# RoyAPTX4869/RaLD

Hardware: AMD Instinct MI355X
Metric: denoising steps/sec (whole node) (higher is better)
Workload: dtype bf16

## Files before the change

### include/rald_hip.h

```cpp
#ifndef RALD_HIP_H
#define RALD_HIP_H
#include <stdint.h>
#ifdef __cplusplus
extern "C" {
#endif

const char* rald_last_error(void);
int rald_version(void);
int rald_build_flags(void);
int64_t rald_debug_f16_saturation_count(int32_t reset);
int rald_debug_poison_lds(void* stream);

typedef struct rald_dit rald_dit;

typedef struct rald_dit_config {
    int32_t n_latents;
    int32_t channels;
    int32_t depth;
    int32_t n_heads;
    int32_t d_head;
    int32_t t_channels;
    int32_t context_dim;
    int32_t n_cond_tokens;
    int32_t with_radar_enc;
    int32_t enc_hidden_ch;
    int32_t enc_radar_ch;
    int32_t radar_r, radar_a, radar_e;
    float sigma_data;
    int32_t qkv_dtype;
} rald_dit_config;

void rald_dit_default_config(rald_dit_config* cfg);
int rald_dit_create(const rald_dit_config* cfg, rald_dit** out);
void rald_dit_destroy(rald_dit* h);
int rald_dit_load_weight(rald_dit* h, const char* name, const float* data, int64_t nelem);
int rald_dit_finalize(rald_dit* h);
int rald_dit_reserve(rald_dit* h, int32_t max_batch);
int64_t rald_dit_workspace_generation(const rald_dit* h);
int rald_dit_set_two_stream_min_batch(rald_dit* h, int32_t min_batch);
int32_t rald_dit_two_stream_min_batch(const rald_dit* h);

int rald_dit_set_sigmas(rald_dit* h, const float* sigmas_host, int32_t n, void* stream);

int64_t rald_dit_cond_cache_bytes(const rald_dit* h, int32_t batch);
int rald_dit_encode_cond_tokens(rald_dit* h, const float* tokens, int32_t batch, void* cond_cache, void* stream);
int rald_dit_encode_cond(rald_dit* h, const float* cube, int32_t batch, float* out_tokens, void* cond_cache, void* stream);

int rald_dit_denoise(rald_dit* h, const float* x, int32_t batch, int32_t sigma_row, int32_t per_sample,
                     const void* cond_cache, float* out, int32_t raw_F, void* stream);

int rald_dit_sample(rald_dit* h, const float* latents, int32_t batch, const void* cond_cache, int32_t num_steps,
                    float sigma_min, float sigma_max, float rho, float* out, void* stream);

int rald_edm_schedule(int32_t num_steps, double sigma_min, double sigma_max, double rho, double S_churn, double S_min, double S_max, float* t,
                      float* t_hat);
int rald_dit_sample_stochastic(rald_dit* h, const float* latents, int32_t batch, const void* cond_cache, int32_t num_steps, double sigma_min,
                               double sigma_max, double rho, double S_churn, double S_min, double S_max, double S_noise, const float* noise,
                               const int64_t* seeds, float* out, void* stream);
int rald_op_philox_normal(const int64_t* seeds, int32_t B, int64_t n_per_sample, int32_t tag, int32_t step, float* out, void* stream);

int rald_dit_profile_begin(rald_dit* h);
int rald_dit_profile_end(rald_dit* h, double* total_ms, int32_t* launches);
int rald_dit_profile_end_kinds(rald_dit* h, double* total_ms4, int32_t* launches4);
int rald_dit_profile_set_kinds(rald_dit* h, uint32_t kind_mask);

typedef struct rald_ae rald_ae;
typedef struct rald_ae_config {
    int32_t dim;
    int32_t num_latents;
    int32_t latent_dim;
    int32_t depth;
    int32_t heads;
    int32_t dim_head;
// ... 187 lines not shown
int rald_op_conv_pack_weights(const float* W, void* out_bf16, int32_t Cout, int32_t Cin, int32_t pad_to, int32_t dgrad, void* stream);
int rald_op_groupnorm(const float* x, const float* gamma, const float* beta, void* y_bf16, double* stats, int32_t B, int32_t S, int32_t C,
                      int32_t swish, void* stream);
int64_t rald_op_groupnorm_bwd_scratch_bytes(int32_t B, int32_t S, int32_t C);
int rald_op_groupnorm_bwd(const float* x, const double* stats, const float* gamma, const float* beta, const void* da, int32_t da_is_bf16, float* dx,
                          void* dx_bf16, float* dgamma, float* dbeta, double* gsum_scratch, int32_t B, int32_t S, int32_t C, int32_t swish,
                          int32_t accumulate, void* stream);
int rald_op_groupnorm_apply(const float* x, const double* stats, const float* gamma, const float* beta, void* y_bf16, int32_t B, int32_t S, int32_t C,
                            int32_t swish, void* stream);
int rald_op_conv_in(const float* cube, int32_t cube_ch, int32_t Cin, const float* W, const float* bias, float* out, int32_t B, int32_t D, int32_t H,
                    int32_t Wd, int32_t Cout, void* stream);
int rald_op_pad_channels(const float* x, void* out_bf16, int64_t M, int32_t C, int32_t Cpad, void* stream);
int rald_op_zero_insert2(const float* dy, void* out_bf16, int32_t B, int32_t OD, int32_t OH, int32_t OW, int32_t C, void* stream);
int rald_op_rowdot(const void* a_bf16, const void* b_bf16, int64_t M, int32_t C, float* out, void* stream);
int rald_op_softmax_rows(const float* S, int64_t ld_s, void* P_bf16, int64_t ld_p, int32_t rows, int32_t n, void* stream);
int rald_op_attn_self_proj(const void* qkv_bf16, int64_t ld, const void* Wo_bf16, float* part, int32_t n_latents, int32_t heads, int32_t batch,
                           void* stream);
int rald_op_xattn_q2_proj(const void* h_bf16, const void* Wq_bf16, const void* Kc_bf16, int64_t ldk, int64_t strideK, const void* Vt_bf16,
                          int64_t ldvt, int64_t strideVt, const void* Wo_bf16, float* part, int32_t M, int32_t n_latents, int32_t heads,
                          int32_t n_keys, float qscale, void* stream);
int rald_op_attn_self_proj_slabs(const void* qkv_bf16, int64_t ld, const void* Wo_bf16, void* part, int32_t n_latents, int32_t heads, int32_t batch,
                                 int32_t part_f16, void* stream);
int rald_op_xattn_q2_proj_slabs(const void* h_bf16, const void* Wq_bf16, const void* Kc_bf16, int64_t ldk, int64_t strideK, const void* Vt_bf16,
                                int64_t ldvt, int64_t strideVt, const void* Wo_bf16, void* part, int32_t M, int32_t n_latents, int32_t heads,
                                int32_t n_keys, float qscale, int32_t part_f16, void* stream);
int rald_op_reduce_resid_ln_slabs(const void* part, int32_t slabs, int64_t slab_stride, const float* bias, float* x, void* h_bf16, int32_t M,
                                  const float* g, const float* b, int64_t gstride, int32_t rows_per_group, float add_one, float eps, int32_t part_f16,
                                  void* stream);
int64_t rald_debug_f16_saturation_attn(int32_t reset);
int rald_op_proj_in(const float* xin, const float* W, float* x, int32_t M, int32_t C, int32_t D, const float* coef, int32_t coef_stride,
                    int32_t rows_per_group, void* stream);
int rald_op_final_norm_proj(const float* x, const float* gamma, const float* beta, const float* Wout, const float* xin, float* out, int32_t M,
                            int32_t D, int32_t C, const float* coef, int32_t coef_stride, int32_t rows_per_group, void* stream);
int rald_op_reduce_resid_ln(const float* part, int32_t slabs, int64_t slab_stride, const float* bias, float* x, void* h_bf16, int32_t M,
                            const float* g, const float* b, int64_t gstride, int32_t rows_per_group, float add_one, float eps, void* stream);
int rald_op_ae_decode_tables(int32_t dim, const float* wq, const float* wk, const float* norm_w, const float* norm_b, const float* wpe,
                             const float* bpe, const float* wfold, float* t2aug_out, uint16_t* l_img_out);
int64_t rald_op_ae_decode_scratch_bytes(int32_t batch, int32_t num_latents);
int rald_op_ae_decode(const float* x, const float* gamma, const float* beta, const float* t2aug, const uint16_t* l_img, const float* basis,
                      float c0, const float* queries, float* out_logits, int32_t batch, int64_t n_queries, int32_t num_latents, int32_t dim,
                      void* scratch, int64_t scratch_bytes, void* stream);
int rald_op_ae_cast_rays(const float* x, const float* gamma, const float* beta, const float* t2aug, const uint16_t* l_img, const float* basis,
                         float c0, const float* origins, const float* dirs, int64_t ray_batch_stride, int32_t n_steps, int32_t n_refine,
                         float* out_t, float* out_logit, int32_t* out_step, float* out_points, int32_t batch, int64_t n_rays,
                         int32_t num_latents, int32_t dim, void* scratch, int64_t scratch_bytes, void* stream);
int rald_op_ae_decode_grad(const float* x, const float* gamma, const float* beta, const float* t2aug, const uint16_t* l_img, const float* basis,
                           float c0, const float* queries, const int64_t* offsets, float* out_logits, float* out_grad, float* out_projected,
                           float max_step, int32_t batch, int64_t n_queries, int32_t num_latents, int32_t dim, void* scratch,
                           int64_t scratch_bytes, void* stream);
int rald_op_ae_encode_tables(int32_t dim, int32_t num_latents, int32_t heads, int32_t mix, const float* const* in, float* const* out);
int rald_op_ae_enc_features(const float* pc, const float* basis, const float* var_factor, void* F_f16, void* G_f16, int32_t batch, int32_t n_points,
                            int32_t rows_per_sample, void* stream);
int rald_op_ae_enc_qproj(const float* xin, const float* X0, float* x, const float* gamma, const float* beta, const float* T1, float* Q,
                         int32_t rows, int32_t num_latents, int32_t dim, void* stream);
int rald_op_attention_f16kv(const float* Q, int64_t ldq, int64_t strideQ, const void* KV_f16, void* O_bf16, int64_t ldo, int64_t strideO, int32_t nq,
                            int32_t nk, int32_t k_rows, int32_t heads, int32_t batch, int32_t ksplit, void* scratch, void* stream);
int rald_op_gemm_mx8(const void* A8, const void* scaleA, int64_t lda, int64_t strideA, int64_t strideSA, const void* B8, const void* scaleB,
                     int64_t ldb, int64_t strideB, int64_t strideSB, void* C, int64_t ldc, int64_t strideC, const float* bias, int32_t M,
                     int32_t N, int32_t K, int32_t batch, float alpha, int32_t epilogue, void* stream);
int rald_op_quantize_mx8(const void* in, int32_t in_is_bf16, int64_t ld_in, void* out_e4m3, int64_t ld_out, void* out_scales_e8m0, int64_t rows,
                         int32_t K, void* stream);
int rald_op_layernorm_mx8(const float* x, void* out_e4m3, void* out_scales_e8m0, int64_t M, int32_t D, const float* g, const float* b,
                          int64_t gstride, int32_t rows_per_group, float add_one, float eps, void* stream);
int rald_op_layernorm(const float* x, void* out_bf16, int32_t M, int32_t D, const float* g, const float* b,
                      int64_t gstride, int32_t rows_per_group, float add_one, float eps, void* stream);
int rald_op_attention(const void* Q, int64_t ldq, int64_t strideQ, const void* K, int64_t ldk, int64_t strideK,
// ... 53 lines not shown
```

### rald_amd/csrc/api.hip

```cpp
#include <cstdlib>
#include <cstring>

#include "ae.h"
#include "dit.h"
#include "lidar.h"
#include "radar_dsp.h"
#include "radar_points.h"

using namespace rald;

struct rald_dit { Dit impl; };
struct rald_ae { Ae impl; };

extern "C" {

const char* rald_last_error(void) { return rald::last_error(); }
int rald_version(void) { return 3; }
int rald_build_flags(void) { return 0; }

int64_t rald_debug_f16_saturation_count(int32_t reset) {
    unsigned a = 0, b = 0;
    if (hipDeviceSynchronize() != hipSuccess) return -1;
    if (f16_saturation_gemm(&a, reset != 0) || f16_saturation_attn(&b, reset != 0)) return -1;
    return (int64_t)a + (int64_t)b;
// ... 18 lines not shown
    rald_dit* h = new rald_dit();
    h->impl.cfg = *cfg;
    int rc = h->impl.create();
    if (rc) { delete h; return rc; }
    *out = h;
    return 0;
}
void rald_dit_destroy(rald_dit* h) {
    if (!h) return;
    (void)hipDeviceSynchronize();
    delete h;
}
int rald_dit_load_weight(rald_dit* h, const char* name, const float* data, int64_t nelem) {
    RALD_CHECK(h && name && data, "rald_dit_load_weight: null argument");
    return h->impl.load_weight(name, data, nelem);
}
int rald_dit_finalize(rald_dit* h) { RALD_CHECK(h, "null handle"); return h->impl.finalize(); }
int rald_dit_reserve(rald_dit* h, int32_t max_batch) {
    RALD_CHECK(h && max_batch >= 1, "rald_dit_reserve: bad argument");
    return h->impl.reserve(max_batch);
}
int64_t rald_dit_workspace_generation(const rald_dit* h) { return h ? h->impl.ws_generation : -1; }
int rald_dit_set_two_stream_min_batch(rald_dit* h, int32_t min_batch) {
    RALD_CHECK(h && min_batch >= 0, "rald_dit_set_two_stream_min_batch: bad argument");
    h->impl.split_min = min_batch;
    if (h->impl.ws_batch > 0) {
        const int B = h->impl.ws_batch;
        h->impl.ws_batch = 0;
        return h->impl.reserve(B);
    }
    return 0;
}
int32_t rald_dit_two_stream_min_batch(const rald_dit* h) { return h ? h->impl.split_min : -1; }
int rald_dit_set_sigmas(rald_dit* h, const float* sigmas_host, int32_t n, void* stream) {
    RALD_CHECK(h && sigmas_host, "rald_dit_set_sigmas: null argument");
    return h->impl.set_sigmas(sigmas_host, n, (hipStream_t)stream);
}
int64_t rald_dit_cond_cache_bytes(const rald_dit* h, int32_t batch) { return h ? h->impl.cond_cache_bytes(batch) : -1; }
int rald_dit_encode_cond_tokens(rald_dit* h, const float* tokens, int32_t batch, void* cond_cache, void* stream) {
    RALD_CHECK(h, "null handle");
    return h->impl.encode_cond_tokens(tokens, batch, cond_cache, (hipStream_t)stream);
}
int rald_dit_encode_cond(rald_dit* h, const float* cube, int32_t batch, float* out_tokens, void* cond_cache, void* stream) {
    RALD_CHECK(h && cube && cond_cache && batch >= 1, "rald_dit_encode_cond: bad argument");
    return h->impl.encode_cond(cube, batch, out_tokens, cond_cache, (hipStream_t)stream);
}
int rald_dit_denoise(rald_dit* h, const float* x, int32_t batch, int32_t sigma_row, int32_t per_sample,
                     const void* cond_cache, float* out, int32_t raw_F, void* stream) {
    RALD_CHECK(h, "null handle");
    return h->impl.denoise(x, batch, sigma_row, per_sample, cond_cache, out, raw_F, (hipStream_t)stream);
}
int rald_dit_sample(rald_dit* h, const float* latents, int32_t batch, const void* cond_cache, int32_t num_steps,
                    float sigma_min, float sigma_max, float rho, float* out, void* stream) {
    RALD_CHECK(h && latents && cond_cache && out && batch >= 1, "rald_dit_sample: bad argument");
    return h->impl.sample(latents, batch, cond_cache, num_steps, sigma_min, sigma_max, rho, out, (hipStream_t)stream);
}
int rald_edm_schedule(int32_t num_steps, double sigma_min, double sigma_max, double rho, double S_churn, double S_min, double S_max, float* t,
                      float* t_hat) {
    return edm_schedule(num_steps, sigma_min, sigma_max, rho, S_churn, S_min, S_max, t, t_hat);
}
int rald_dit_sample_stochastic(rald_dit* h, const float* latents, int32_t batch, const void* cond_cache, int32_t num_steps, double sigma_min,
                               double sigma_max, double rho, double S_churn, double S_min, double S_max, double S_noise, const float* noise,
                               const int64_t* seeds, float* out, void* stream) {
    RALD_CHECK(h && latents && cond_cache && out && batch >= 1, "rald_dit_sample_stochastic: bad argument");
    return h->impl.sample_stochastic(latents, batch, cond_cache, num_steps, sigma_min, sigma_max, rho, S_churn, S_min, S_max, S_noise, noise,
                                     seeds, out, (hipStream_t)stream);
// ... 711 lines not shown
int rald_op_ae_enc_features(const float* pc, const float* basis, const float* var_factor, void* F_f16, void* G_f16, int32_t batch, int32_t n_points,
                            int32_t rows_per_sample, void* stream) {
    RALD_CHECK(pc && basis && var_factor && F_f16 && G_f16, "rald_op_ae_enc_features: null pointer");
    RALD_CHECK(batch >= 1 && n_points >= 1, "rald_op_ae_enc_features: batch and n_points must be at least 1");
    RALD_CHECK(rows_per_sample >= n_points && rows_per_sample % 64 == 0,
               "rald_op_ae_enc_features: rows_per_sample must be a multiple of 64 and at least n_points");
    RALD_CHECK((uintptr_t)F_f16 % 16 == 0 && (uintptr_t)G_f16 % 16 == 0, "rald_op_ae_enc_features: F and G must be 16-byte aligned");
    return ae_enc_features(pc, basis, var_factor, F_f16, G_f16, batch, n_points, rows_per_sample, (hipStream_t)stream);
}
int rald_op_ae_enc_qproj(const float* xin, const float* X0, float* x, const float* gamma, const float* beta, const float* T1, float* Q,
                         int32_t rows, int32_t num_latents, int32_t dim, void* stream) {
    RALD_CHECK(X0 && x && gamma && beta && T1 && Q, "rald_op_ae_enc_qproj: null pointer (only xin may be null)");
    RALD_CHECK(rows >= 1, "rald_op_ae_enc_qproj: rows must be at least 1");
    RALD_CHECK(num_latents >= 1, "rald_op_ae_enc_qproj: num_latents must be at least 1");
    RALD_CHECK(dim == 256 || dim == 512, "rald_op_ae_enc_qproj: dim must be 256 or 512");
    return ae_enc_qproj(xin, X0, x, gamma, beta, T1, Q, rows, num_latents, dim, (hipStream_t)stream);
}
int rald_op_ae_encode_tables(int32_t dim, int32_t num_latents, int32_t heads, int32_t mix, const float* const* in, float* const* out) {
    RALD_CHECK(in && out && dim >= 64 && num_latents >= 1 && heads >= 1, "rald_op_ae_encode_tables: bad argument");
    for (int i = 0; i < 18; ++i) RALD_CHECK(in[i] || (!mix && i >= 2 && i <= 11 && i != 9), "rald_op_ae_encode_tables: null input tensor");
    const int I = heads * 64;
    std::vector<float> Rf, Q1, T4, X0, T1, T3, c3;
    RALD_TRY(rald::ae_encode_tables(dim, I, num_latents, heads, mix != 0, in[0], in[1], in[2], in[3], in[4], in[5], in[6], in[7], in[8], in[9], in[10], in[11],
                                    in[12], in[13], in[14], in[15], in[16], in[17], Rf, Q1, T4, X0, T1, T3, c3));
    const std::vector<float>* v[7] = {&Rf, &Q1, &T4, &X0, &T1, &T3, &c3};
    for (int i = 0; i < 7; ++i)
        if (out[i] && !v[i]->empty()) memcpy(out[i], v[i]->data(), v[i]->size() * 4);
    return 0;
}
int rald_op_proj_in(const float* xin, const float* W, float* x, int32_t M, int32_t C, int32_t D, const float* coef, int32_t coef_stride,
                    int32_t rows_per_group, void* stream) {
    RALD_CHECK(xin && W && x && coef && M >= 1 && rows_per_group >= 1, "rald_op_proj_in: bad argument");
    return proj_in(xin, W, x, M, C, D, coef, coef_stride, rows_per_group, (hipStream_t)stream);
}
int rald_op_final_norm_proj(const float* x, const float* gamma, const float* beta, const float* Wout, const float* xin, float* out, int32_t M,
                            int32_t D, int32_t C, const float* coef, int32_t coef_stride, int32_t rows_per_group, void* stream) {
    RALD_CHECK(x && gamma && beta && Wout && xin && out && coef && M >= 1 && rows_per_group >= 1, "rald_op_final_norm_proj: bad argument");
    return final_norm_proj(x, gamma, beta, Wout, xin, out, M, D, C, coef, coef_stride, rows_per_group, (hipStream_t)stream);
}
int rald_op_attn_self_proj(const void* qkv_bf16, int64_t ld, const void* Wo_bf16, float* part, int32_t n_latents, int32_t heads, int32_t batch,
                           void* stream) {
    return attn_self_proj((const bf16*)qkv_bf16, ld, (const bf16*)Wo_bf16, part, n_latents, heads, batch, (hipStream_t)stream);
}
int rald_op_xattn_q2_proj(const void* h_bf16, const void* Wq_bf16, const void* Kc_bf16, int64_t ldk, int64_t strideK, const void* Vt_bf16,
                          int64_t ldvt, int64_t strideVt, const void* Wo_bf16, float* part, int32_t M, int32_t n_latents, int32_t heads,
                          int32_t n_keys, float qscale, void* stream) {
    return xattn_q2_proj((const bf16*)h_bf16, (const bf16*)Wq_bf16, (const bf16*)Kc_bf16, ldk, strideK, (const bf16*)Vt_bf16, ldvt, strideVt,
                         (const bf16*)Wo_bf16, part, M, n_latents, heads, n_keys, qscale, (hipStream_t)stream);
}
int rald_op_reduce_resid_ln(const float* part, int32_t slabs, int64_t slab_stride, const float* bias, float* x, void* h_bf16, int32_t M,
                            const float* g, const float* b, int64_t gstride, int32_t rows_per_group, float add_one, float eps, void* stream) {
    return reduce_resid_ln(part, slabs, slab_stride, bias, x, (bf16*)h_bf16, M, g, b, gstride, rows_per_group, add_one, eps, (hipStream_t)stream);
}
int rald_op_attn_self_proj_slabs(const void* qkv_bf16, int64_t ld, const void* Wo_bf16, void* part, int32_t n_latents, int32_t heads, int32_t batch,
                                 int32_t part_f16, void* stream) {
    return attn_self_proj((const bf16*)qkv_bf16, ld, (const bf16*)Wo_bf16, (float*)part, n_latents, heads, batch, (hipStream_t)stream, part_f16 != 0);
}
int rald_op_xattn_q2_proj_slabs(const void* h_bf16, const void* Wq_bf16, const void* Kc_bf16, int64_t ldk, int64_t strideK, const void* Vt_bf16,
                                int64_t ldvt, int64_t strideVt, const void* Wo_bf16, void* part, int32_t M, int32_t n_latents, int32_t heads,
                                int32_t n_keys, float qscale, int32_t part_f16, void* stream) {
    return xattn_q2_proj((const bf16*)h_bf16, (const bf16*)Wq_bf16, (const bf16*)Kc_bf16, ldk, strideK, (const bf16*)Vt_bf16, ldvt, strideVt,
                         (const bf16*)Wo_bf16, (float*)part, M, n_latents, heads, n_keys, qscale, (hipStream_t)stream, part_f16 != 0);
}
int rald_op_reduce_resid_ln_slabs(const void* part, int32_t slabs, int64_t slab_stride, const float* bias, float* x, void* h_bf16, int32_t M,
                                  const float* g, const float* b, int64_t gstride, int32_t rows_per_group, float add_one, float eps, int32_t part_f16,
                                  void* stream) {
// ... 109 lines not shown
```

### rald_amd/csrc/dit.h

```cpp
#pragma once
#include <map>
#include <set>
#include <string>
#include <vector>

#include "../../include/rald_hip.h"
#include "common.h"
#include "kernels.h"

namespace rald {

const char* last_error();

struct DeviceArena {
    std::vector<void*> ptrs;
    void* alloc(size_t bytes, bool zero);
    void release(void* p);
    ~DeviceArena();
};

struct BlobHeader { uint32_t magic; int32_t batch; int32_t flag; uint32_t cfg_hash; int64_t bytes; uint32_t pad[10]; };
static_assert(sizeof(BlobHeader) == 64, "blob header is 64 bytes");
constexpr int BLOB_HEADER_BYTES = 64;
struct BlobRegistry {
// ... 45 lines not shown
    bf16 *w_k2_all = nullptr, *w_v2_all = nullptr;
    float *w_mod = nullptr, *b_mod = nullptr;
    float *w_t0 = nullptr, *b_t0 = nullptr, *w_t1 = nullptr, *b_t1 = nullptr;
    float *w_in = nullptr, *w_out = nullptr, *norm_g = nullptr, *norm_b = nullptr, *coef_raw = nullptr;
    bf16* w_out_hl = nullptr;
    int* d_geglu_map = nullptr;
    RadarEncoder radar;
    std::set<std::string> expected, loaded;
    bool finalized = false;
    struct SigmaTable {
        std::string key;
        std::vector<float> host;
        int n = 0, cap = 0;
        float *sigma = nullptr, *coef = nullptr, *cnoise = nullptr, *pe = nullptr, *temb0 = nullptr, *temb = nullptr, *mod = nullptr;
    };
    SigmaTable tables[3];
    int build_table(SigmaTable& t, const float* sig, int n, hipStream_t st);
    int64_t mod_row() const { return (int64_t)cfg.depth * 3 * 2 * D; }
    int64_t ws_generation = 0;
    int ws_batch = 0;
    struct Work {
        float* x = nullptr;
        float* part = nullptr;
        bf16 *h = nullptr, *qk = nullptr, *o = nullptr, *q2 = nullptr, *g = nullptr;
        unsigned char *h8 = nullptr, *hs = nullptr;
        unsigned char *g8 = nullptr, *gs = nullptr;
        int rows = 0;
    };
    Work wk[2];
    int alloc_work(Work& w, size_t M);
    void free_work(Work& w);
    float *ws_xcur = nullptr, *ws_xeul = nullptr, *ws_den = nullptr, *ws_dcur = nullptr;
    bf16* ws_tok = nullptr;
    int split_min = 256;
    hipStream_t side = nullptr;
    hipEvent_t ev_fork = nullptr, ev_join = nullptr;
    bool fork_pending = false;
    int split_sizes(int B, int& b0) const { b0 = ((B / 2 + 32) / 64) * 64; return split_min > 0 && B >= split_min && b0 >= 64 && b0 < B; }
    static constexpr uint32_t COND_MAGIC = 0x52414c44u;
    static constexpr int COND_HEADER_BYTES = BLOB_HEADER_BYTES;
    BlobRegistry cond_registry;
    uint32_t cfg_hash() const;
    BlobHeader cond_header(int B) const;

    static constexpr int PROF_KINDS = 4;
    bool prof_on = false;
    unsigned prof_mask = 0xf;
    std::vector<hipEvent_t> prof_ev;
    std::vector<int> prof_kind;
    int prof_used = 0;
    int profile_begin();
    int profile_end(double* total_ms, int* launches);
    int profile_end_kinds(double* total_ms, int* launches);
    ~Dit();

    int create();
    int load_weight(const std::string& name, const float* data, int64_t nelem);
    int finalize();
    int reserve(int B);
    int set_sigmas(const float* sig, int n, hipStream_t st);
    int64_t cond_cache_bytes(int B) const;
    bool cond_fold(int B) const;
    int encode_cond_tokens(const float* tokens, int B, void* cache, hipStream_t st);
    int encode_cond(const float* cube, int B, float* out_tokens, void* cache, hipStream_t st);
    int denoise(const float* x, int B, int sigma_row, int per_sample, const void* cache, float* out, int raw_F, hipStream_t st, int slot = 0);
    int denoise_range(const float* x, int Bfull, int b0, int Bn, int sigma_row, int per_sample, const void* cache, float* out, int raw_F,
// ... 9 lines not shown
```

### rald_amd/csrc/dit.hip

```cpp
#include "dit.h"

#include <cmath>
#include <cstdio>
#include <cstdlib>
#include <cstring>

namespace rald {

static thread_local std::string g_err;
void set_error(const std::string& msg) { g_err = msg; }
const char* last_error() { return g_err.c_str(); }

void* DeviceArena::alloc(size_t bytes, bool zero) {
    void* p = nullptr;
    if (bytes == 0) bytes = 16;
    if (hipMalloc(&p, bytes) != hipSuccess) return nullptr;
    if (zero) {
        (void)hipMemset(p, 0, bytes);
        (void)hipStreamSynchronize(nullptr);
    }
    ptrs.push_back(p);
    return p;
}
void DeviceArena::release(void* p) {
// ... 493 lines not shown
    const bf16* Vtc = Vtc0 + (size_t)b0 * L * D * T;
    const float scale = 1.0f / sqrtf((float)cfg.d_head);
    const float qscale = scale * 1.4426950408889634f;
    const bool mx1 = cfg.qkv_dtype >= 1, mx2 = cfg.qkv_dtype >= 2;

    auto timed_launch = [&](int kind, auto&& launch) -> int {
        const bool timed = timed_ok && !mx1 && prof_on && ((prof_mask >> kind) & 1u) && prof_used + 2 <= (int)prof_ev.size();
        if (timed) RALD_HIP(hipEventRecord(prof_ev[prof_used], st));
        RALD_TRY(launch());
        if (timed) { RALD_HIP(hipEventRecord(prof_ev[prof_used + 1], st)); prof_kind[prof_used / 2] = kind; prof_used += 2; }
        return 0;
    };
    auto proj = [&](bool mx8, GemmArgs g, const unsigned char* W8, const unsigned char* SW, int epi) -> int {
        if (!mx8) return gemm_nt(g, epi, st);
        Mx8Args a;
        a.g = g; a.g.A = nullptr; a.g.B = nullptr;
        a.A8 = ws_h8; a.SA = ws_hs; a.B8 = W8; a.SB = SW; a.strideSA = 0; a.strideSB = 0;
        return gemm_mx8(a, epi, st);
    };
    auto resid_args = [&](const bf16* A, int64_t ld, const bf16* W, const float* bias, int K, const float* mnext, bool mx8) {
        GemmLnArgs g = gemm_ln_args(A, ld, W, ld, bias, ws_x, mx8 ? nullptr : ws_h, mnext, mnext ? mnext + D : nullptr, gstride, NL, 1.0f, M, K);
        if (mx8 && mnext) { g.h8 = ws_h8; g.hs = ws_hs; }
        return g;
    };
    auto resid_ln = [&](const bf16* A, int64_t ld, const bf16* W, const float* bias, int K, const float* mnext, bool mx8) {
        return resid_gemm_ln(resid_args(A, ld, W, bias, K, mnext, mx8), D, ws_part, st);
    };
    const bool fold = cond_fold(Bfull);
    const bool small = !mx1 && small_m_fused(M, NL, cfg.n_heads, D, T);
    RALD_CHECK(!fold || !small, "dit: a folded condition cache cannot feed the small-batch kernels (internal)");
    const bf16* Gt0 = Vtc0 + (size_t)2 * Bfull * T * L * D;
    const bf16* Gt = Gt0 + (size_t)b0 * L * D * D;
    const bf16* Ut = Gt0 + (size_t)Bfull * L * D * D + (size_t)b0 * L * D * D;
    RALD_TRY(proj_in(x, w_in, ws_x, M, C, D, coef, cstride, NL, st));
    RALD_TRY(mx1 ? layernorm_mod_mx8(ws_x, ws_h8, ws_hs, M, D, mod, mod + D, gstride, NL, 1.0f, 1e-5f, st)
                 : layernorm_mod(ws_x, ws_h, M, D, mod, mod + D, gstride, NL, 1.0f, 1e-5f, st));
    for (int li = 0; li < L; ++li) {
        const Layer& l = layers[li];
        const float* m2 = mod + (int64_t)(li * 3 + 1) * 2 * D;
        const float* m3 = mod + (int64_t)(li * 3 + 2) * 2 * D;
        GemmArgs qkv = gemm_args(ws_h, D, l.w_qk, D, ws_qk, 3 * D, nullptr, M, 3 * D, D);
        qkv.alpha = qscale; qkv.alpha_ncols = D;
        RALD_TRY(proj(mx1, qkv, l.q8_qk, l.s8_qk, EPI_BF16));
        if (small) {
            RALD_TRY(attn_self_proj(ws_qk, 3 * D, l.w_o, ws_part, NL, cfg.n_heads, B, st, true));
            RALD_TRY(reduce_resid_ln(ws_part, cfg.n_heads, (int64_t)M * D, l.b_o, ws_x, ws_h, M, m2, m2 + D, gstride, NL, 1.0f, 1e-5f, st, true));
            RALD_TRY(xattn_q2_proj(ws_h, l.w_q2, Kc + (size_t)li * D, (int64_t)L * D, (int64_t)T * L * D, Vtc + (size_t)li * D * T, T, (int64_t)L * D * T,
                                   l.w_o2, ws_part, M, NL, cfg.n_heads, T, qscale, st, true));
            RALD_TRY(reduce_resid_ln(ws_part, cfg.n_heads, (int64_t)M * D, l.b_o2, ws_x, ws_h, M, m3, m3 + D, gstride, NL, 1.0f, 1e-5f, st, true));
        } else {
            RALD_TRY(attention_d64(self_attn_args(ws_qk, ws_o, NL, D, cfg.n_heads, B, scale), st));
            RALD_TRY(timed_launch(1, [&] { return resid_ln(ws_o, D, l.w_o, l.b_o, D, m2, mx1); }));
            if (fold) {
                GemmArgs p1 = gemm_args(ws_h, D, Gt + (size_t)li * D * D, D, ws_q2, D, nullptr, NL, D, D);
                p1.batch = B; p1.strideA = (int64_t)NL * D; p1.strideB = (int64_t)L * D * D; p1.strideC = (int64_t)NL * D;
                RALD_TRY(gemm_nt(p1, EPI_SOFTMAX64, st));
                GemmLnArgs g = resid_args(ws_q2, D, Ut + (size_t)li * D * D, l.b_o2, D, m3, false);
                g.strideW = (int64_t)L * D * D; g.w_rows = NL;
                RALD_TRY(timed_launch(2, [&] { return resid_gemm_ln(g, D, ws_part, st); }));
            } else {
                GemmArgs q2 = gemm_args(ws_h, D, l.w_q2, D, ws_q2, D, nullptr, M, D, D);
                q2.alpha = qscale;
                RALD_TRY(proj(mx1, q2, l.q8_q2, l.s8_q2, EPI_BF16));
                AttnArgs a2;
                a2.Q = ws_q2; a2.ldq = D; a2.strideQ = (int64_t)NL * D;
                a2.K = Kc + (size_t)li * D; a2.ldk = (int64_t)L * D; a2.strideK = (int64_t)T * L * D;
                a2.Vt = Vtc + (size_t)li * D * T; a2.ldvt = T; a2.strideVt = (int64_t)L * D * T;
                a2.O = ws_o; a2.ldo = D; a2.strideO = (int64_t)NL * D;
                a2.nq = NL; a2.nk = T; a2.k_rows = T; a2.heads = cfg.n_heads; a2.batch = B; a2.scale = scale; a2.q_prescaled = 1;
                RALD_TRY(attention_d64(a2, st));
                if (mx1 && fork_pending && timed_ok) { RALD_HIP(hipEventRecord(ev_fork, st)); fork_pending = false; }
                RALD_TRY(resid_ln(ws_o, D, l.w_o2, l.b_o2, D, m3, mx2));
            }
        }
        if (fork_pending && timed_ok) { RALD_HIP(hipEventRecord(ev_fork, st)); fork_pending = false; }
        const bool ff2_mx = cfg.qkv_dtype == 3 && M % 256 == 0 && M >= 4096 && gemm_resid_ln_pays(M, 4 * D);
        GemmArgs f1 = gemm_args(ws_h, D, l.w_ff1, D, ws_g, 4 * D, l.b_ff1, M, 8 * D, D);
        if (ff2_mx) { f1.out8 = ws_g8; f1.outs = ws_gs; }
        RALD_TRY(timed_launch(0, [&] { return proj(mx2, f1, l.q8_ff1, l.s8_ff1, EPI_GEGLU); }));
        const float* m1_next = (li + 1 < L) ? mod + (int64_t)((li + 1) * 3) * 2 * D : nullptr;
        if (ff2_mx) {
            GemmLnArgs g = resid_args(nullptr, 4 * D, nullptr, l.b_ff2, 4 * D, m1_next ? m1_next : m3, true);
            g.A8 = ws_g8; g.SA = ws_gs; g.W8 = l.q8_ff2; g.SW = l.s8_ff2;
            RALD_TRY(resid_gemm_ln(g, D, ws_part, st));
        } else {
            RALD_TRY(timed_launch(3, [&] { return resid_ln(ws_g, 4 * D, l.w_ff2, l.b_ff2, 4 * D, m1_next, mx1); }));
        }
    }
    RALD_TRY(final_norm_proj(ws_x, norm_g, norm_b, w_out, x, out, M, D, C, coef, cstride, NL, st, w_out_hl));
    return 0;
}

int Dit::profile_begin() {
    if (prof_ev.empty()) {
        prof_ev.resize(2 * 16384);
        prof_kind.assign(16384, 0);
        for (auto& e : prof_ev) RALD_HIP(hipEventCreate(&e));
    }
    prof_used = 0;
    prof_on = true;
    return 0;
}
int Dit::profile_end_kinds(double* total_ms, int* launches) {
    prof_on = false;
    for (int k = 0; k < PROF_KINDS; ++k) { total_ms[k] = 0.0; launches[k] = 0; }
    for (int i = 0; i + 1 < prof_used; i += 2) {
        RALD_HIP(hipEventSynchronize(prof_ev[i + 1]));
        float ms = 0.f;
        RALD_HIP(hipEventElapsedTime(&ms, prof_ev[i], prof_ev[i + 1]));
        const int k = prof_kind[i / 2];
        total_ms[k] += ms;
        launches[k] += 1;
    }
    prof_used = 0;
    return 0;
}
int Dit::profile_end(double* total_ms, int* launches) {
    double ms[PROF_KINDS];
    int n[PROF_KINDS];
// ... 83 lines not shown
```

### rald_amd/csrc/gemm_ln.hip

```cpp
#include <cstdlib>
#include <type_traits>
#include <utility>

#include "common.h"
#include "kernels.h"
#include "gemm_tile.h"
#include "mx8.h"

namespace rald {

template <int BM, int WM, int WN>
struct LnEpiLds {
    static constexpr int NT = 512 / (16 * WN);
    static constexpr int ROWB_F = NT * 16 * 4, STRIDE_F = ROWB_F + 16;
    static constexpr int ROWB_H = NT * 16 * 2, STRIDE_H = ROWB_H + 16;
    static constexpr int PATCH = 16 * STRIDE_F;
    static constexpr int RED_OFF = WM * WN * PATCH;
    static constexpr int VEC_OFF = RED_OFF + BM * WN * 8;
    static constexpr int BYTES = VEC_OFF + 3 * 512 * 4;
};

template <int... Q, typename F>
__device__ __forceinline__ void unrolled(std::integer_sequence<int, Q...>, F&& f) { (f(std::integral_constant<int, Q>{}), ...); }
template <int N, typename F>
// ... 137 lines not shown
                    if (mm < a.M) {
                        *reinterpret_cast<uint2*>(a.h8 + mc * BN + col) = *reinterpret_cast<const uint2*>(q8);
                        if ((pc & 3) == 0) a.hs[mc * (BN / 32) + col / 32] = sc;
                    }
                } else if (mm < a.M) {
                    typedef unsigned int nt_u32x4 __attribute__((ext_vector_type(4)));
                    if (nt_io) __builtin_nontemporal_store(nt_u32x4{v.x, v.y, v.z, v.w}, reinterpret_cast<nt_u32x4*>(a.h + (int64_t)mm * BN + nb + pc * 8));
                    else *reinterpret_cast<uint4*>(a.h + (int64_t)mm * BN + nb + pc * 8) = v;
                }
            }
        }
    }
}

template <int BM, int WM, int WN, bool MX, bool GU>
__device__ __forceinline__ void gemm_resid_ln_body(const GemmLnArgs& a) {
    constexpr int BN = 512, NSTAGE = 2, BK = 64;
    constexpr int WAVES = WM * WN;
    constexpr int MT = BM / (16 * WM);
    constexpr int NT = BN / (16 * WN);
    constexpr int ROWB = 128;
    constexpr int RPP = 1024 / ROWB;
    constexpr int CA = BM / RPP / WAVES;
    constexpr int CB = BN / RPP / WAVES;
    static_assert(CA >= 1 && CB >= 1 && BM % (RPP * WAVES) == 0 && BN % (RPP * WAVES) == 0 && MT >= 1 && NT >= 1, "tile/wave split");
    constexpr int STAGE_BYTES = (BM + BN) * ROWB;
    static_assert(LnEpiLds<BM, WM, WN>::BYTES <= NSTAGE * STAGE_BYTES, "epilogue scratch (patches, red, bias | g | b) must fit in the staging buffers");
    extern __shared__ __attribute__((aligned(16))) unsigned char smem[];

    const int tid = threadIdx.x;
    const int lane = tid & 63;
    const int wave = __builtin_amdgcn_readfirstlane(tid >> 6);
    const int wm = wave / WN, wn = wave % WN;
    int mtile = blockIdx.x;
    if (a.strideW != 0) {
        const int tg = a.w_rows / BM, ngroups = (int)gridDim.x / (tg > 0 ? tg : 1);
        if (tg >= 1 && tg < 8 && ngroups * tg == (int)gridDim.x && (ngroups & 7) == 0) {
            const int slot = (int)blockIdx.x >> 3;
            mtile = ((slot / tg) * 8 + ((int)blockIdx.x & 7)) * tg + slot % tg;
        }
    }
    const int m0 = mtile * BM;
    constexpr int ESZ = MX ? 1 : 2;
    const unsigned char* A0 = MX ? a.A8 : reinterpret_cast<const unsigned char*>(a.A);
    const unsigned char* W0 = MX ? a.W8 : reinterpret_cast<const unsigned char*>(a.W + (int64_t)(m0 / a.w_rows) * a.strideW);

    typedef float nt_f32x4 __attribute__((ext_vector_type(4)));
    const bool nt_io_ = (a.nt_io & 1) != 0;
    f32x4 acc[MT][NT];
    const int nk = MX ? a.K / 128 : a.K / BK;
    const int fr = lane & 15, fq = lane >> 4;
    if constexpr (MX) {
        Mx8Loop<BM, BN, WM, WN> L;
        L.begin(acc, A0, a.lda, a.SA, m0, a.M, W0, a.ldw, a.SW, 0, BN, a.K, smem, wave, lane);
        for (int kt = 0; kt < nk; ++kt) L.step(acc, kt, kt & 1, (kt + 1) & 1, smem, wave, lane);
    } else {
#pragma unroll
    for (int i = 0; i < MT; ++i)
#pragma unroll
        for (int j = 0; j < NT; ++j) acc[i][j] = f32x4{0.f, 0.f, 0.f, 0.f};
    constexpr int XP = MT * NT / 8;
    static_assert(MT * NT % 8 == 0, "x pieces per k-step");
    nt_f32x4 xt[XP];
    const int mb_ = m0 + wm * (BM / WM), nb_ = wn * (BN / WN);
    const unsigned char* xbase = reinterpret_cast<const unsigned char*>(a.x) + (int64_t)mb_ * BN * 4;
    unsigned xoff[MT];
#pragma unroll
    for (int i = 0; i < MT; ++i) {
        int r = i * 16 + fr;
        r = mb_ + r < a.M ? r : a.M - 1 - mb_;
        xoff[i] = (unsigned)r * (BN * 4) + (unsigned)(nb_ + 4 * fq) * 4;
    }
// ... 237 lines not shown
```

### rald_amd/csrc/kernels.h

```cpp
#pragma once
#include <cstdlib>
#include <vector>

#include "common.h"

namespace rald {

enum { GEMM_NT_STORE = 64 };
enum { EPI_BF16 = 0, EPI_F32 = 1, EPI_RESID = 2, EPI_GEGLU = 3,
       EPI_SOFTMAX64 = 4,
       EPI_F16S = 5 };
struct GemmArgs {
    const bf16* A; int64_t lda; int64_t strideA;
    const bf16* B; int64_t ldb; int64_t strideB;
    void* C;       int64_t ldc; int64_t strideC;
    const float* bias;
    int M, N, K, batch;
    float alpha;
    int alpha_ncols;
    int flags;
    int batch2 = 1;
    int64_t strideA2 = 0, strideB2 = 0, strideC2 = 0;
    unsigned char *out8 = nullptr, *outs = nullptr;
};
// ... 5 lines not shown
    oc = (int64_t)b1 * a.strideC + (int64_t)b2 * a.strideC2;
}
#endif
int gemm_nt(const GemmArgs& a, int epi, hipStream_t st);
int gemm_nt_256_test(const GemmArgs& a, int epi, int persistent, int max_workgroups, hipStream_t st);
int gemm_nt_256_batched_test(const GemmArgs& a, int epi, int persistent, int max_workgroups, hipStream_t st);
int f16_saturation_gemm(unsigned* count, bool reset);
int f16_saturation_attn(unsigned* count, bool reset);
inline bool gemm_f16s_ok(int M, int N, int batch) {
    const int64_t w128 = (int64_t)((M + 127) / 128) * ((N + 127) / 128) * batch, w64 = (int64_t)((M + 63) / 64) * ((N + 63) / 64) * batch;
    return w128 >= 192 || w64 <= 256;
}
inline GemmArgs gemm_args(const bf16* A, int64_t lda, const bf16* B, int64_t ldb, void* C, int64_t ldc,
                          const float* bias, int M, int N, int K) {
    GemmArgs g;
    g.A = A; g.lda = lda; g.strideA = 0; g.B = B; g.ldb = ldb; g.strideB = 0;
    g.C = C; g.ldc = ldc; g.strideC = 0; g.bias = bias; g.M = M; g.N = N; g.K = K; g.batch = 1; g.alpha = 1.f; g.alpha_ncols = 1 << 30; g.flags = 0;
    return g;
}

struct GemmLnArgs {
    const bf16* A; int64_t lda;
    const bf16* W; int64_t ldw;
    const float* bias;
    float* x;
    bf16* h;
    unsigned char* h8 = nullptr;
    unsigned char* hs = nullptr;
    int nt_io = 1;
    const unsigned char *A8 = nullptr, *SA = nullptr, *W8 = nullptr, *SW = nullptr;
    const float* g; const float* b; int64_t gstride; int rows_per_group; float add_one, eps;
    int M, K;
    int64_t strideW = 0; int w_rows = 1 << 30;
};
int gemm_resid_ln(const GemmLnArgs& a, hipStream_t st);
inline bool gemm_resid_ln_pays(int M, int K = 512) { (void)K; return M >= 16384; }
inline GemmLnArgs gemm_ln_args(const bf16* A, int64_t lda, const bf16* W, int64_t ldw, const float* bias, float* x, bf16* h,
                               const float* g, const float* b, int64_t gstride, int rows_per_group, float add_one, int M, int K) {
    GemmLnArgs a;
    a.A = A; a.lda = lda; a.W = W; a.ldw = ldw; a.bias = bias; a.x = x; a.h = h;
    a.g = g; a.b = b; a.gstride = gstride; a.rows_per_group = rows_per_group; a.add_one = add_one; a.eps = 1e-5f; a.M = M; a.K = K;
    return a;
}
int resid_gemm_ln(const GemmLnArgs& a, int n, float* scratch, hipStream_t st);

int patches27(const float* cube, int cube_ch, bf16* out, int B, int D, int H, int Wd, hipStream_t st);
int gemm_tn(const bf16* A, int64_t lda, const bf16* B, int64_t ldb, float* C, int64_t ldc, float* colsum, int M, int N1, int N2, hipStream_t st,
            float* workspace = nullptr, int64_t workspace_floats = 0);
int64_t gemm_tn_workspace_floats(int M, int N1, int N2);
int conv3d_wgrad_tn(const bf16* dy, const bf16* x, float* dW, float* dbias, int B, int ID, int IH, int IW, int Cin, int Cout, int stride, int pad,
                    hipStream_t st, float* workspace = nullptr, int64_t workspace_floats = 0);
int64_t conv3d_wgrad_workspace_floats(int B, int ID, int IH, int IW, int Cin, int Cout, int stride, int pad);

int layernorm_mod(const float* x, bf16* out, int M, int D, const float* g, const float* b,
                  int64_t gstride, int rows_per_group, float add_one, float eps, hipStream_t st);
int proj_in(const float* xin, const float* W, float* x, int M, int C, int D, const float* coef,
            int coef_stride, int rows_per_group, hipStream_t st);
int final_norm_proj(const float* x, const float* gamma, const float* beta, const float* Wout,
                    const float* xin, float* out, int M, int D, int C, const float* coef,
                    int coef_stride, int rows_per_group, hipStream_t st, const bf16* Whl = nullptr);
int split_hi_lo(const float* w, bf16* out, int n, hipStream_t st);

struct AttnArgs {
    const bf16* Q;  int64_t ldq,  strideQ;
    const bf16* K;  int64_t ldk,  strideK;
    const bf16* Vt; int64_t ldvt, strideVt;
    const bf16* V = nullptr; int64_t ldv = 0, strideV = 0;
    int ksplit = 1; float* part = nullptr;
    bf16* O;        int64_t ldo,  strideO;
    int nq, nk, heads, batch;
    int k_rows;
    float scale;
    int q_prescaled;
    int f16 = 0; const float* Qf = nullptr;
    int hsk = 64;
    int v_padded = 0;
};
int attention_d64(const AttnArgs& a, hipStream_t st);
inline AttnArgs self_attn_args(const bf16* qkv, bf16* O, int n, int inner, int heads, int batch, float scale) {
    AttnArgs a;
    a.Q = qkv; a.ldq = 3 * inner; a.strideQ = (int64_t)n * 3 * inner;
    a.K = qkv + inner; a.ldk = 3 * inner; a.strideK = (int64_t)n * 3 * inner;
    a.Vt = nullptr; a.ldvt = 0; a.strideVt = 0;
    a.V = qkv + 2 * inner; a.ldv = 3 * inner; a.strideV = (int64_t)n * 3 * inner;
    a.O = O; a.ldo = inner; a.strideO = (int64_t)n * inner;
    a.nq = n; a.nk = n; a.k_rows = n; a.heads = heads; a.batch = batch; a.scale = scale; a.q_prescaled = 1;
    return a;
}
int attention_pick_ksplit(int nq, int nk, int heads, int batch);
inline int64_t attention_split_scratch_bytes(int ksplit, int nq, int heads, int batch) { return (int64_t)ksplit * batch * heads * nq * 66 * 4; }
// ... 225 lines not shown
```

### rald_amd/csrc/norm.hip

```cpp
#include "common.h"
#include "kernels.h"

namespace rald {

template <int VPL>
__global__ __launch_bounds__(256) void layernorm_mod_kernel(const float* __restrict__ x, bf16* __restrict__ out,
                                                            int M, const float* __restrict__ g, const float* __restrict__ b,
                                                            int64_t gstride, int rows_per_group, float add_one, float eps) {
    constexpr int NC = VPL / 4;
    constexpr int D = VPL * 64;
    const int lane = threadIdx.x & 63;
    const int row = blockIdx.x * 4 + (threadIdx.x >> 6);
    if (row >= M) return;
    const float4* xr = reinterpret_cast<const float4*>(x + (int64_t)row * D);
    float4 v[NC];
    float s = 0.f;
#pragma unroll
    for (int c = 0; c < NC; ++c) {
        v[c] = xr[lane + 64 * c];
        s += v[c].x + v[c].y + v[c].z + v[c].w;
    }
    const float mean = wave_sum(s) * (1.0f / D);
    float q = 0.f;
#pragma unroll
    for (int c = 0; c < NC; ++c) {
        float dx = v[c].x - mean, dy = v[c].y - mean, dz = v[c].z - mean, dw = v[c].w - mean;
        q += dx * dx + dy * dy + dz * dz + dw * dw;
    }
    const float rstd = rsqrtf(wave_sum(q) * (1.0f / D) + eps);
    const int64_t goff = (int64_t)(row / rows_per_group) * gstride;
    const float4* gr = reinterpret_cast<const float4*>(g + goff);
    const float4* br = reinterpret_cast<const float4*>(b + goff);
// ... 171 lines not shown
#pragma unroll
        for (int r = 0; r < 16; ++r) {
            const int m = m0 + 16 * half + r;
            if (m < M) x[(int64_t)m * D + n0 + n] = acc[r];
        }
    }
}

template <int C>
static int launch_proj_in(const float* xin, const float* W, float* x, int M, int D, const float* coef, int coef_stride, int rows_per_group,
                          hipStream_t st) {
    hipLaunchKernelGGL(proj_in_kernel<C>, dim3(cdiv(M, 32), D / 256), dim3(256), 0, st, xin, W, x, M, D, coef, coef_stride, rows_per_group);
    RALD_HIP(hipGetLastError());
    return 0;
}
int proj_in(const float* xin, const float* W, float* x, int M, int C, int D, const float* coef,
            int coef_stride, int rows_per_group, hipStream_t st) {
    RALD_CHECK(C >= 1 && C <= 64, "proj_in: latent channels must be in [1,64]");
    RALD_CHECK(D % 256 == 0, "proj_in: D must be a multiple of 256");
    if (M > 4096) {
        switch (C) {
            case 4: return launch_proj_in<4>(xin, W, x, M, D, coef, coef_stride, rows_per_group, st);
            case 8: return launch_proj_in<8>(xin, W, x, M, D, coef, coef_stride, rows_per_group, st);
            case 16: return launch_proj_in<16>(xin, W, x, M, D, coef, coef_stride, rows_per_group, st);
            case 32: return launch_proj_in<32>(xin, W, x, M, D, coef, coef_stride, rows_per_group, st);
            default: break;
        }
    }
    hipLaunchKernelGGL(proj_in_small_kernel, dim3(cdiv(M, 8)), dim3(256), 0, st, xin, W, x, M, C, D, coef, coef_stride, rows_per_group);
    RALD_HIP(hipGetLastError());
    return 0;
}

template <int VPL>
__global__ __launch_bounds__(256) void final_norm_proj_kernel(const float* __restrict__ x, const float* __restrict__ gamma,
                                                              const float* __restrict__ beta, const float* __restrict__ Wout,
                                                              const float* __restrict__ xin, float* __restrict__ out, int M, int C,
                                                              const float* __restrict__ coef, int coef_stride, int rows_per_group) {
    constexpr int NC = VPL / 4;
    constexpr int D = VPL * 64;
    const int lane = threadIdx.x & 63;
    const int row = blockIdx.x * 4 + (threadIdx.x >> 6);
    if (row >= M) return;
    const float4* xr = reinterpret_cast<const float4*>(x + (int64_t)row * D);
    float4 v[NC];
    float s = 0.f;
#pragma unroll
    for (int c = 0; c < NC; ++c) {
        v[c] = xr[lane + 64 * c];
        s += v[c].x + v[c].y + v[c].z + v[c].w;
    }
    const float mean = wave_sum(s) * (1.0f / D);
    float q = 0.f;
#pragma unroll
    for (int c = 0; c < NC; ++c) {
        float dx = v[c].x - mean, dy = v[c].y - mean, dz = v[c].z - mean, dw = v[c].w - mean;
        q += dx * dx + dy * dy + dz * dz + dw * dw;
    }
    const float rstd = rsqrtf(wave_sum(q) * (1.0f / D) + 1e-5f);
#pragma unroll
    for (int c = 0; c < NC; ++c) {
        float4 gg = reinterpret_cast<const float4*>(gamma)[lane + 64 * c];
        float4 bb = reinterpret_cast<const float4*>(beta)[lane + 64 * c];
        v[c].x = (v[c].x - mean) * rstd * gg.x + bb.x;
        v[c].y = (v[c].y - mean) * rstd * gg.y + bb.y;
        v[c].z = (v[c].z - mean) * rstd * gg.z + bb.z;
// ... 172 lines not shown
```

Baseline: 6122.

## Fuse proj_in with first modulated layernorm and reverse FF2 tile order

Adds a fused proj_in+layernorm kernel for C=32, D=512 that keeps the input projection weights in LDS, computes each projected row and writes both the fp32 residual and the modulated bf16 LN output in one pass. This removes a separate layernorm launch and one full reread of the residual stream. It also adds a reversed M-tile ordering option for the FF2 residual GEMM+LN, likely to reuse data the previous kernel left in cache. Both are on by default through a new route mask, and a setter is exposed to turn them off.

```diff
diff --git a/include/rald_hip.h b/include/rald_hip.h
--- a/include/rald_hip.h
+++ b/include/rald_hip.h
@@ -39,6 +39,8 @@
 int64_t rald_dit_workspace_generation(const rald_dit* h);
 int rald_dit_set_two_stream_min_batch(rald_dit* h, int32_t min_batch);
 int32_t rald_dit_two_stream_min_batch(const rald_dit* h);
+int rald_dit_set_routes(rald_dit* h, uint32_t mask);
+int32_t rald_dit_routes(const rald_dit* h);
 
 int rald_dit_set_sigmas(rald_dit* h, const float* sigmas_host, int32_t n, void* stream);
 
@@ -292,6 +294,9 @@
                     int32_t rows_per_group, void* stream);
 int rald_op_final_norm_proj(const float* x, const float* gamma, const float* beta, const float* Wout, const float* xin, float* out, int32_t M,
                             int32_t D, int32_t C, const float* coef, int32_t coef_stride, int32_t rows_per_group, void* stream);
+int rald_op_proj_in_ln(const float* xin, const float* W, float* x, void* h_bf16, int32_t M, int32_t C, int32_t D, const float* coef,
+                       int32_t coef_stride, const float* g, const float* b, int64_t gstride, int32_t rows_per_group, float add_one, float eps,
+                       void* stream);
 int rald_op_reduce_resid_ln(const float* part, int32_t slabs, int64_t slab_stride, const float* bias, float* x, void* h_bf16, int32_t M,
                             const float* g, const float* b, int64_t gstride, int32_t rows_per_group, float add_one, float eps, void* stream);
 int rald_op_ae_decode_tables(int32_t dim, const float* wq, const float* wk, const float* norm_w, const float* norm_b, const float* wpe,
diff --git a/rald_amd/csrc/api.hip b/rald_amd/csrc/api.hip
--- a/rald_amd/csrc/api.hip
+++ b/rald_amd/csrc/api.hip
@@ -74,6 +74,12 @@
     return 0;
 }
 int32_t rald_dit_two_stream_min_batch(const rald_dit* h) { return h ? h->impl.split_min : -1; }
+int rald_dit_set_routes(rald_dit* h, uint32_t mask) {
+    RALD_CHECK(h && mask < 4u, "rald_dit_set_routes: bad argument");
+    h->impl.routes = mask;
+    return 0;
+}
+int32_t rald_dit_routes(const rald_dit* h) { return h ? (int32_t)h->impl.routes : -1; }
 int rald_dit_set_sigmas(rald_dit* h, const float* sigmas_host, int32_t n, void* stream) {
     RALD_CHECK(h && sigmas_host, "rald_dit_set_sigmas: null argument");
     return h->impl.set_sigmas(sigmas_host, n, (hipStream_t)stream);
@@ -851,6 +857,12 @@
                     int32_t rows_per_group, void* stream) {
     RALD_CHECK(xin && W && x && coef && M >= 1 && rows_per_group >= 1, "rald_op_proj_in: bad argument");
     return proj_in(xin, W, x, M, C, D, coef, coef_stride, rows_per_group, (hipStream_t)stream);
+}
+int rald_op_proj_in_ln(const float* xin, const float* W, float* x, void* h_bf16, int32_t M, int32_t C, int32_t D, const float* coef,
+                       int32_t coef_stride, const float* g, const float* b, int64_t gstride, int32_t rows_per_group, float add_one, float eps,
+                       void* stream) {
+    RALD_CHECK(xin && W && x && h_bf16 && coef && g && b && M >= 1 && rows_per_group >= 1, "rald_op_proj_in_ln: bad argument");
+    return proj_in_ln(xin, W, x, (bf16*)h_bf16, M, C, D, coef, coef_stride, g, b, gstride, rows_per_group, add_one, eps, (hipStream_t)stream);
 }
 int rald_op_final_norm_proj(const float* x, const float* gamma, const float* beta, const float* Wout, const float* xin, float* out, int32_t M,
                             int32_t D, int32_t C, const float* coef, int32_t coef_stride, int32_t rows_per_group, void* stream) {
diff --git a/rald_amd/csrc/dit.h b/rald_amd/csrc/dit.h
--- a/rald_amd/csrc/dit.h
+++ b/rald_amd/csrc/dit.h
@@ -101,6 +101,8 @@
     void free_work(Work& w);
     float *ws_xcur = nullptr, *ws_xeul = nullptr, *ws_den = nullptr, *ws_dcur = nullptr;
     bf16* ws_tok = nullptr;
+    static constexpr unsigned ROUTE_PROJ_IN_LN = 1, ROUTE_REV_FF2 = 2;
+    unsigned routes = ROUTE_PROJ_IN_LN | ROUTE_REV_FF2;
     int split_min = 256;
     hipStream_t side = nullptr;
     hipEvent_t ev_fork = nullptr, ev_join = nullptr;
diff --git a/rald_amd/csrc/dit.hip b/rald_amd/csrc/dit.hip
--- a/rald_amd/csrc/dit.hip
+++ b/rald_amd/csrc/dit.hip
@@ -549,9 +549,13 @@
     const bf16* Gt0 = Vtc0 + (size_t)2 * Bfull * T * L * D;
     const bf16* Gt = Gt0 + (size_t)b0 * L * D * D;
     const bf16* Ut = Gt0 + (size_t)Bfull * L * D * D + (size_t)b0 * L * D * D;
-    RALD_TRY(proj_in(x, w_in, ws_x, M, C, D, coef, cstride, NL, st));
-    RALD_TRY(mx1 ? layernorm_mod_mx8(ws_x, ws_h8, ws_hs, M, D, mod, mod + D, gstride, NL, 1.0f, 1e-5f, st)
-                 : layernorm_mod(ws_x, ws_h, M, D, mod, mod + D, gstride, NL, 1.0f, 1e-5f, st));
+    if (!mx1 && (routes & ROUTE_PROJ_IN_LN) && proj_in_ln_ok(C, D)) {
+        RALD_TRY(proj_in_ln(x, w_in, ws_x, ws_h, M, C, D, coef, cstride, mod, mod + D, gstride, NL, 1.0f, 1e-5f, st));
+    } else {
+        RALD_TRY(proj_in(x, w_in, ws_x, M, C, D, coef, cstride, NL, st));
+        RALD_TRY(mx1 ? layernorm_mod_mx8(ws_x, ws_h8, ws_hs, M, D, mod, mod + D, gstride, NL, 1.0f, 1e-5f, st)
+                     : layernorm_mod(ws_x, ws_h, M, D, mod, mod + D, gstride, NL, 1.0f, 1e-5f, st));
+    }
     for (int li = 0; li < L; ++li) {
         const Layer& l = layers[li];
         const float* m2 = mod + (int64_t)(li * 3 + 1) * 2 * D;
@@ -601,7 +605,9 @@
             g.A8 = ws_g8; g.SA = ws_gs; g.W8 = l.q8_ff2; g.SW = l.s8_ff2;
             RALD_TRY(resid_gemm_ln(g, D, ws_part, st));
         } else {
-            RALD_TRY(timed_launch(3, [&] { return resid_ln(ws_g, 4 * D, l.w_ff2, l.b_ff2, 4 * D, m1_next, mx1); }));
+            GemmLnArgs g = resid_args(ws_g, 4 * D, l.w_ff2, l.b_ff2, 4 * D, m1_next, mx1);
+            g.rev_m = (routes & ROUTE_REV_FF2) != 0;
+            RALD_TRY(timed_launch(3, [&] { return resid_gemm_ln(g, D, ws_part, st); }));
         }
     }
     RALD_TRY(final_norm_proj(ws_x, norm_g, norm_b, w_out, x, out, M, D, C, coef, cstride, NL, st, w_out_hl));
diff --git a/rald_amd/csrc/gemm_ln.hip b/rald_amd/csrc/gemm_ln.hip
--- a/rald_amd/csrc/gemm_ln.hip
+++ b/rald_amd/csrc/gemm_ln.hip
@@ -193,12 +193,13 @@
     const int lane = tid & 63;
     const int wave = __builtin_amdgcn_readfirstlane(tid >> 6);
     const int wm = wave / WN, wn = wave % WN;
-    int mtile = blockIdx.x;
+    const int bid = a.rev_m * ((int)gridDim.x - 1) + (1 - 2 * a.rev_m) * (int)blockIdx.x;
+    int mtile = bid;
     if (a.strideW != 0) {
         const int tg = a.w_rows / BM, ngroups = (int)gridDim.x / (tg > 0 ? tg : 1);
         if (tg >= 1 && tg < 8 && ngroups * tg == (int)gridDim.x && (ngroups & 7) == 0) {
-            const int slot = (int)blockIdx.x >> 3;
-            mtile = ((slot / tg) * 8 + ((int)blockIdx.x & 7)) * tg + slot % tg;
+            const int slot = bid >> 3;
+            mtile = ((slot / tg) * 8 + (bid & 7)) * tg + slot % tg;
         }
     }
     const int m0 = mtile * BM;
diff --git a/rald_amd/csrc/kernels.h b/rald_amd/csrc/kernels.h
--- a/rald_amd/csrc/kernels.h
+++ b/rald_amd/csrc/kernels.h
@@ -61,6 +61,7 @@
     const float* g; const float* b; int64_t gstride; int rows_per_group; float add_one, eps;
     int M, K;
     int64_t strideW = 0; int w_rows = 1 << 30;
+    int rev_m = 0;
 };
 int gemm_resid_ln(const GemmLnArgs& a, hipStream_t st);
 inline bool gemm_resid_ln_pays(int M, int K = 512) { (void)K; return M >= 16384; }
@@ -85,6 +86,9 @@
                   int64_t gstride, int rows_per_group, float add_one, float eps, hipStream_t st);
 int proj_in(const float* xin, const float* W, float* x, int M, int C, int D, const float* coef,
             int coef_stride, int rows_per_group, hipStream_t st);
+bool proj_in_ln_ok(int C, int D);
+int proj_in_ln(const float* xin, const float* W, float* x, bf16* h, int M, int C, int D, const float* coef, int coef_stride, const float* g,
+               const float* b, int64_t gstride, int rows_per_group, float add_one, float eps, hipStream_t st);
 int final_norm_proj(const float* x, const float* gamma, const float* beta, const float* Wout,
                     const float* xin, float* out, int M, int D, int C, const float* coef,
                     int coef_stride, int rows_per_group, hipStream_t st, const bf16* Whl = nullptr);
diff --git a/rald_amd/csrc/norm.hip b/rald_amd/csrc/norm.hip
--- a/rald_amd/csrc/norm.hip
+++ b/rald_amd/csrc/norm.hip
@@ -1,3 +1,5 @@
+#include <algorithm>
+
 #include "common.h"
 #include "kernels.h"
 
@@ -235,6 +237,137 @@
     return 0;
 }
 
+__device__ __forceinline__ void ln_mod_row512(const float4 (&v)[2], const float4 (&gg)[2], const float4 (&bb)[2], int lane, bf16* __restrict__ orow_,
+                                              float add_one, float eps, bool store) {
+#pragma clang fp contract(off)
+    float s = 0.f;
+#pragma unroll
+    for (int c = 0; c < 2; ++c) s += v[c].x + v[c].y + v[c].z + v[c].w;
+    const float mean = wave_sum(s) * (1.0f / 512);
+    float4 d[2];
+    float q = 0.f;
+#pragma unroll
+    for (int c = 0; c < 2; ++c) {
+        d[c] = make_float4(v[c].x - mean, v[c].y - mean, v[c].z - mean, v[c].w - mean);
+        q += fmaf(d[c].w, d[c].w, fmaf(d[c].z, d[c].z, fmaf(d[c].x, d[c].x, d[c].y * d[c].y)));
+    }
+    const float rstd = rsqrtf(fmaf(wave_sum(q), 1.0f / 512, eps));
+    bf16x4* orow = reinterpret_cast<bf16x4*>(orow_);
+#pragma unroll
+    for (int c = 0; c < 2; ++c) {
+        const bf16x4 o = pack4(fmaf(add_one + gg[c].x, d[c].x * rstd, bb[c].x), fmaf(add_one + gg[c].y, d[c].y * rstd, bb[c].y),
+                               fmaf(add_one + gg[c].z, d[c].z * rstd, bb[c].z), fmaf(add_one + gg[c].w, d[c].w * rstd, bb[c].w));
+        if (store) orow[lane + 64 * c] = o;
+    }
+}
+__device__ __forceinline__ void ln_mod_load512(float4 (&gg)[2], float4 (&bb)[2], int lane, const float* __restrict__ g, const float* __restrict__ b) {
+#pragma unroll
+    for (int c = 0; c < 2; ++c) {
+        gg[c] = reinterpret_cast<const float4*>(g)[lane + 64 * c];
+        bb[c] = reinterpret_cast<const float4*>(b)[lane + 64 * c];
+    }
+}
+struct ProjInLnArgs {
+    const float* xin; const float* W; float* x; bf16* h;
+    const float* coef; int coef_stride;
+    const float* g; const float* b; int64_t gstride; int rows_per_group;
+    float add_one, eps;
+    int M;
+};
+template <int RW>
+__global__ __launch_bounds__(256) void proj_in_ln_kernel(ProjInLnArgs a) {
+    constexpr int C = 32, D = 512, R = 4 * RW;
+    extern __shared__ __attribute__((aligned(16))) unsigned char smem[];
+    float* const swt = reinterpret_cast<float*>(smem);
+    float* const sx = swt + C * D;
+    const int lane = threadIdx.x & 63, wave = threadIdx.x >> 6;
+    for (int n = threadIdx.x; n < D; n += 256) {
+        const float4* wr = reinterpret_cast<const float4*>(a.W + (int64_t)n * C);
+#pragma unroll
+        for (int c4 = 0; c4 < C / 4; ++c4) {
+            const float4 w = wr[c4];
+            swt[(4 * c4 + 0) * D + n] = w.x; swt[(4 * c4 + 1) * D + n] = w.y; swt[(4 * c4 + 2) * D + n] = w.z; swt[(4 * c4 + 3) * D + n] = w.w;
+        }
+    }
+    float* const sxw = sx + wave * RW * C;
+    const int ntiles = (a.M + R - 1) / R;
+    auto load_rows = [&](int tile) {
+        const int r0 = tile * R + wave * RW, m = r0 + lane / (C / 4);
+        float4 v = make_float4(0.f, 0.f, 0.f, 0.f);
+        if (lane < RW * (C / 4) && m < a.M) {
+            v = reinterpret_cast<const float4*>(a.xin + (int64_t)r0 * C)[lane];
+            const float cin = a.coef[(int64_t)(m / a.rows_per_group) * a.coef_stride + 0];
+            v.x = v.x * cin; v.y = v.y * cin; v.z = v.z * cin; v.w = v.w * cin;
+        }
+        return v;
+    };
+    float4 xrows = load_rows(blockIdx.x);
+    for (int tile = blockIdx.x; tile < ntiles; tile += gridDim.x) {
+        const int r0 = tile * R + wave * RW;
+        __syncthreads();
+        if (lane < RW * (C / 4)) reinterpret_cast<float4*>(sxw)[lane] = xrows;
+        __syncthreads();
+        if (tile + (int)gridDim.x < ntiles) xrows = load_rows(tile + gridDim.x);
+        const int rfirst = r0 < a.M ? r0 : a.M - 1, rlast = r0 + RW - 1 < a.M ? r0 + RW - 1 : a.M - 1;
+        const int64_t goff0 = (int64_t)(rfirst / a.rows_per_group) * a.gstride;
+        const bool one_group = goff0 == (int64_t)(rlast / a.rows_per_group) * a.gstride;
+        float4 gg[2], bb[2];
+        ln_mod_load512(gg, bb, lane, a.g + goff0, a.b + goff0);
+        f32x2 acc[RW][4];
+#pragma unroll
+        for (int r = 0; r < RW; ++r)
+#pragma unroll
+            for (int j = 0; j < 4; ++j) acc[r][j] = f32x2{0.f, 0.f};
+#pragma unroll 2
+        for (int c4 = 0; c4 < C / 4; ++c4) {
+            float4 wa[4], wb[4];
+#pragma unroll
+            for (int k = 0; k < 4; ++k) {
+                wa[k] = reinterpret_cast<const float4*>(swt + (4 * c4 + k) * D)[lane];
+                wb[k] = reinterpret_cast<const float4*>(swt + (4 * c4 + k) * D)[lane + 64];
+            }
+#pragma unroll
+            for (int r = 0; r < RW; ++r) {
+                const float4 s4 = reinterpret_cast<const float4*>(sxw + r * C)[c4];
+                const float s[4] = {s4.x, s4.y, s4.z, s4.w};
+#pragma unroll
+                for (int k = 0; k < 4; ++k) {
+                    const f32x2 sk = f32x2{s[k], s[k]};
+                    acc[r][0] = __builtin_elementwise_fma(sk, f32x2{wa[k].x, wa[k].y}, acc[r][0]);
+                    acc[r][1] = __builtin_elementwise_fma(sk, f32x2{wa[k].z, wa[k].w}, acc[r][1]);
+                    acc[r][2] = __builtin_elementwise_fma(sk, f32x2{wb[k].x, wb[k].y}, acc[r][2]);
+                    acc[r][3] = __builtin_elementwise_fma(sk, f32x2{wb[k].z, wb[k].w}, acc[r][3]);
+                }
+            }
+        }
+#pragma unroll
+        for (int r = 0; r < RW; ++r) {
+            const int row = r0 + r;
+            const bool live = row < a.M;
+            const float4 v[2] = {make_float4(acc[r][0][0], acc[r][0][1], acc[r][1][0], acc[r][1][1]),
+                                 make_float4(acc[r][2][0], acc[r][2][1], acc[r][3][0], acc[r][3][1])};
+            float4* xr = reinterpret_cast<float4*>(a.x + (int64_t)row * D);
+            if (live) { xr[lane] = v[0]; xr[lane + 64] = v[1]; }
+            if (!one_group && live) {
+                const int64_t goff = (int64_t)(row / a.rows_per_group) * a.gstride;
+                ln_mod_load512(gg, bb, lane, a.g + goff, a.b + goff);
+            }
+            ln_mod_row512(v, gg, bb, lane, a.h + (int64_t)row * D, a.add_one, a.eps, live);
+        }
+    }
+}
+
+bool proj_in_ln_ok(int C, int D) { return C == 32 && D == 512; }
+int proj_in_ln(const float* xin, const float* W, float* x, bf16* h, int M, int C, int D, const float* coef, int coef_stride, const float* g,
+               const float* b, int64_t gstride, int rows_per_group, float add_one, float eps, hipStream_t st) {
+    RALD_CHECK(proj_in_ln_ok(C, D), "proj_in_ln: 32 latent channels and D = 512 only");
+    RALD_CHECK(M >= 1 && rows_per_group >= 1, "proj_in_ln: bad sizes");
+    const ProjInLnArgs a{xin, W, x, h, coef, coef_stride, g, b, gstride, rows_per_group, add_one, eps, M};
+    static bool raised8 = false, raised2 = false;
+    if (M > 4096) return launch_dyn_lds(proj_in_ln_kernel<8>, raised8, dim3(std::min(cdiv(M, 32), 512)), 256, (32 * 512 + 4 * 8 * 32) * 4, st, a);
+    return launch_dyn_lds(proj_in_ln_kernel<2>, raised2, dim3(cdiv(M, 8)), 256, (32 * 512 + 4 * 2 * 32) * 4, st, a);
+}
+
 template <int VPL>
 __global__ __launch_bounds__(256) void final_norm_proj_kernel(const float* __restrict__ x, const float* __restrict__ gamma,
                                                               const float* __restrict__ beta, const float* __restrict__ Wout,
```

Result: no change. 6140 (median of 6 runs) (+0.3%).
